# NVIDIA/CUDALibrarySamples

Hardware: NVIDIA H100
Metric: csr_spmv_fp64_effective_hbm_bandwidth (higher is better)
Workload: dtype f64

## Files before the change

### cudalibrarysamples_b200/csrc/spmv_csr_flat.cu

```cuda
#include "spmv_common.cuh"
#include "config.h"
#include "../../include/b200spmv.h"

namespace b200 {

#ifndef B200_FLAT_MIN_CTAS
#define B200_FLAT_MIN_CTAS 10
#endif
#ifndef B200_FLAT_BATCH
#define B200_FLAT_BATCH 4
#endif
#ifndef B200_FLAT_STEPS
#define B200_FLAT_STEPS 8
#endif
#ifndef B200_FLAT_KBLOOP
#define B200_FLAT_KBLOOP (B200_FLAT_STEPS > 8)
#endif
#ifndef B200_FLAT_NZPRE
#define B200_FLAT_NZPRE 0
#endif
constexpr int PLAN_STEPS = 8;
constexpr int PLAN_CHUNK = 32 * PLAN_STEPS;
constexpr int FLAT_STEPS = B200_FLAT_STEPS;
constexpr int FLAT_CHUNK = 32 * FLAT_STEPS;
static_assert(FLAT_STEPS % PLAN_STEPS == 0 && FLAT_STEPS <= 32, "a warp chunk is 1, 2 or 4 plan chunks");
#ifndef B200_FLAT_WARPS
#define B200_FLAT_WARPS 4
#endif
constexpr int FLAT_WARPS = B200_FLAT_WARPS;
constexpr int FLAT_BLOCK = 32 * FLAT_WARPS;
constexpr int FLAT_CTA_NNZ = FLAT_CHUNK * FLAT_WARPS;
constexpr int FLAT_CTA_WORDS = FLAT_CTA_NNZ / 32;
constexpr int FLAT_PAD_NNZ = 2048;
static_assert(FLAT_PAD_NNZ % FLAT_CTA_NNZ == 0, "FLAT_WARPS x FLAT_STEPS must divide 64");
constexpr int FLAT_BATCH64 = B200_FLAT_BATCH;
#ifdef B200_FLAT_BATCH32
constexpr int FLAT_BATCH32 = B200_FLAT_BATCH32;
#else
constexpr int FLAT_BATCH32 = (2 * B200_FLAT_BATCH <= B200_FLAT_STEPS) ? 2 * B200_FLAT_BATCH : B200_FLAT_BATCH;
#endif
constexpr int SCAN_ITEMS = 2048;
static_assert(FLAT_STEPS % FLAT_BATCH64 == 0 && FLAT_STEPS % FLAT_BATCH32 == 0, "steps per chunk must be a multiple of the batch");

struct FlatPlan {
    unsigned* endmask;
    int*      chunk_run;
    int*      nzrow;
    double*   cta_first;
    double*   cta_last;
    int*      cta_flags;
    int*      ctl;
    int*      scratch;
};

static inline size_t flat_align(size_t v) { return (v + 255) / 256 * 256; }
static inline int64_t flat_num_ctas(int64_t nnz) { return (nnz + FLAT_CTA_NNZ - 1) / FLAT_CTA_NNZ; }
static inline int64_t flat_num_chunks_padded(int64_t nnz) { return (nnz + FLAT_PAD_NNZ - 1) / FLAT_PAD_NNZ * (FLAT_PAD_NNZ / PLAN_CHUNK); }

static size_t flat_layout(int64_t rows, int64_t nnz, void* ws, FlatPlan* p) {
    const size_t nchunks = (size_t)flat_num_chunks_padded(nnz);
    const size_t nctas = nchunks;
    const size_t nscan = (size_t)((rows > (int64_t)nchunks ? rows : (int64_t)nchunks) / SCAN_ITEMS + 2);
    size_t o = 0;
    const size_t o_mask = o;  o = flat_align(o + nchunks * PLAN_STEPS * sizeof(unsigned));
    const size_t o_crun = o;  o = flat_align(o + (nchunks + 1) * sizeof(int));
    const size_t o_nzr  = o;  o = flat_align(o + ((size_t)rows + 2 + 32) * sizeof(int));
    const size_t o_cf   = o;  o = flat_align(o + nctas * sizeof(double));
    const size_t o_cl   = o;  o = flat_align(o + nctas * sizeof(double));
    const size_t o_fl   = o;  o = flat_align(o + nctas * sizeof(int));
    const size_t o_ctl  = o;  o = flat_align(o + 64);
    const size_t o_scr  = o;  o = flat_align(o + nscan * sizeof(int));
    if (p) {
        char* b = (char*)ws;
        p->endmask = (unsigned*)(b + o_mask); p->chunk_run = (int*)(b + o_crun); p->nzrow = (int*)(b + o_nzr);
        p->cta_first = (double*)(b + o_cf); p->cta_last = (double*)(b + o_cl); p->cta_flags = (int*)(b + o_fl);
        p->ctl = (int*)(b + o_ctl); p->scratch = (int*)(b + o_scr);
    }
    return o;
}

__global__ void flat_mark_ends_kernel(const int* __restrict__ off, int base, int64_t rows, unsigned* __restrict__ endmask) {
    for (int64_t r = (int64_t)blockIdx.x * blockDim.x + threadIdx.x; r < rows; r += (int64_t)gridDim.x * blockDim.x) {
        const int b = off[r] - base, e = off[r + 1] - base;
        if (e > b) atomicOr(endmask + ((e - 1) >> 5), 1u << ((e - 1) & 31));
    }
}

struct RowNonEmpty {
    const int* off;
    __device__ __forceinline__ int operator()(int64_t r) const { return off[r + 1] > off[r] ? 1 : 0; }
};
struct ChunkEnds {
    const unsigned* endmask;
    __device__ __forceinline__ int operator()(int64_t c) const {
        int n = 0;
#pragma unroll
        for (int k = 0; k < PLAN_STEPS; k++) n += __popc(endmask[c * PLAN_STEPS + k]);
        return n;
    }
};

template <typename V>
__global__ void __launch_bounds__(256) scan_block_sums_kernel(V value, int64_t n, int* __restrict__ block_sums) {
    __shared__ int sw[8];
    const int64_t i0 = (int64_t)blockIdx.x * SCAN_ITEMS;
    int s = 0;
    for (int k = threadIdx.x; k < SCAN_ITEMS; k += 256) {
        const int64_t i = i0 + k;
        s += i < n ? value(i) : 0;
    }
#pragma unroll
    for (int o = 16; o > 0; o >>= 1) s += __shfl_xor_sync(0xffffffffu, s, o);
    if ((threadIdx.x & 31) == 0) sw[threadIdx.x >> 5] = s;
    __syncthreads();
    if (threadIdx.x == 0) {
        int t = 0;
#pragma unroll
        for (int w = 0; w < 8; w++) t += sw[w];
        block_sums[blockIdx.x] = t;
    }
}

__global__ void __launch_bounds__(1024) scan_of_block_sums_kernel(int* __restrict__ block_sums, int64_t nb, int* __restrict__ total) {
    __shared__ int sw[32];
    __shared__ int carry;
    if (threadIdx.x == 0) carry = 0;
    __syncthreads();
    for (int64_t i0 = 0; i0 < nb; i0 += 1024) {
        const int64_t i = i0 + threadIdx.x;
        const int v = i < nb ? block_sums[i] : 0;
        int incl = v;
#pragma unroll
        for (int o = 1; o < 32; o <<= 1) { const int t = __shfl_up_sync(0xffffffffu, incl, o); if ((threadIdx.x & 31) >= o) incl += t; }
        if ((threadIdx.x & 31) == 31) sw[threadIdx.x >> 5] = incl;
        __syncthreads();
        if (threadIdx.x < 32) {
            const int w = sw[threadIdx.x];
            int wi = w;
#pragma unroll
            for (int o = 1; o < 32; o <<= 1) { const int t = __shfl_up_sync(0xffffffffu, wi, o); if (threadIdx.x >= o) wi += t; }
            sw[threadIdx.x] = wi - w;
        }
        __syncthreads();
        const int excl = carry + sw[threadIdx.x >> 5] + incl - v;
        if (i < nb) block_sums[i] = excl;
        __syncthreads();
        if (threadIdx.x == 1023) carry = excl + v;
        __syncthreads();
    }
    if (threadIdx.x == 0) *total = carry;
}

template <typename V, typename E>
__global__ void __launch_bounds__(256) scan_emit_kernel(V value, E emit, int64_t n, const int* __restrict__ block_sums) {
    __shared__ int sw[8];
    __shared__ int carry;
    if (threadIdx.x == 0) carry = block_sums[blockIdx.x];
    __syncthreads();
    const int64_t i0 = (int64_t)blockIdx.x * SCAN_ITEMS;
    for (int k0 = 0; k0 < SCAN_ITEMS; k0 += 256) {
        const int64_t i = i0 + k0 + threadIdx.x;
        const int v = i < n ? value(i) : 0;
        int incl = v;
#pragma unroll
        for (int o = 1; o < 32; o <<= 1) { const int t = __shfl_up_sync(0xffffffffu, incl, o); if ((threadIdx.x & 31) >= o) incl += t; }
        if ((threadIdx.x & 31) == 31) sw[threadIdx.x >> 5] = incl;
        __syncthreads();
        int woff = 0;
#pragma unroll
        for (int w = 0; w < 8; w++) woff += w < (int)(threadIdx.x >> 5) ? sw[w] : 0;
        const int excl = carry + woff + incl - v;
        if (i < n) emit(i, excl, v);
        __syncthreads();
        if (threadIdx.x == 255) carry = excl + v;
        __syncthreads();
    }
}

struct EmitNzRow {
    int* nzrow;
    __device__ __forceinline__ void operator()(int64_t r, int rank, int v) const { if (v) nzrow[rank + 1] = (int)r; }
};
struct EmitChunkRun {
    int* chunk_run;
    __device__ __forceinline__ void operator()(int64_t c, int before, int) const { chunk_run[c] = before; }
};

__global__ void flat_finish_kernel(FlatPlan p, int64_t rows, int64_t nchunks, int64_t nwords) {
    const int nruns = p.ctl[0];
    if (blockIdx.x == 0 && threadIdx.x == 0) {
        p.nzrow[0] = -1;
        p.nzrow[nruns + 1] = (int)rows;
        p.chunk_run[nchunks] = nruns;
        p.ctl[2] = (int)nwords;
    }
    int quiet = 0;
    for (int64_t w = (int64_t)blockIdx.x * blockDim.x + threadIdx.x; w < nwords; w += (int64_t)gridDim.x * blockDim.x)
        quiet += p.endmask[w] == 0u;
#pragma unroll
    for (int o = 16; o > 0; o >>= 1) quiet += __shfl_xor_sync(0xffffffffu, quiet, o);
    if ((threadIdx.x & 31) == 0 && quiet) atomicAdd(p.ctl + 1, quiet);
}

template <typename T>
struct FlatArgs {
    const int* off;
    const int* col;
    const T*   val;
    const T*   x;
    T*         y;
    int        base;
    int        rows;
    int        nnz;
    Scalars<T> s;
    FlatPlan   plan;
};

template <typename T>
__device__ __forceinline__ T flat_allsum(T v) {
#pragma unroll
    for (int o = 16; o > 0; o >>= 1) v += __shfl_xor_sync(0xffffffffu, v, o);
    return v;
}

template <typename T>
__device__ __forceinline__ void flat_store_y(T* yp, T alpha, T v, T beta) {
    T old = T(0);
    if (beta != T(0)) old = *yp;
    *yp = alpha * v + beta * old;
}

template <typename T>
__global__ void __launch_bounds__(FLAT_BLOCK, B200_FLAT_MIN_CTAS) csr_flat_kernel(const FlatArgs<T> a) {
    __shared__ T   sFirst[FLAT_WARPS], sLast[FLAT_WARPS];
    __shared__ int sFrow[FLAT_WARPS];
    __shared__ int sArrived;
    if (threadIdx.x == 0) sArrived = 0;
    __syncthreads();

    const int lane = (int)threadIdx.x & 31, warp = (int)threadIdx.x >> 5;
    const long long c = (long long)blockIdx.x * FLAT_WARPS + warp;
    const long long c0 = c * FLAT_CHUNK;
    const bool active = c0 < a.nnz;
    const T alpha = a.s.a(), beta = a.s.b();
    T   acc = T(0), first = T(0), last = T(0);
    int frow = -1;

    if (active) {
        const int n0 = (int)c0, n1 = min(n0 + FLAT_CHUNK, a.nnz);
        const unsigned mreg = lane < FLAT_STEPS ? __ldg(a.plan.endmask + c * FLAT_STEPS + lane) : 0u;
        int run = __ldg(a.plan.chunk_run + c * (FLAT_STEPS / PLAN_STEPS));
#if B200_FLAT_NZPRE
        const int run0 = run;
        const int nzw = __ldg(a.plan.nzrow + run0 + 1 + lane);
#endif
        const int* colp = a.col + n0;
        const T*   valp = a.val + n0;
        const T*   xp = a.x - a.base;
        constexpr int FLAT_BATCH = sizeof(T) == 8 ? FLAT_BATCH64 : FLAT_BATCH32;
        int cc[FLAT_BATCH];
        T   vv[FLAT_BATCH];
        auto issue = [&](int kb) {
#pragma unroll
            for (int k = 0; k < FLAT_BATCH; k++) {
                const int e = (kb + k) * 32 + lane;
                const bool live = n0 + e < n1;
                cc[k] = live ? ldg_stream(colp + e) : a.base;
                vv[k] = live ? ldg_stream(valp + e) : T(0);
            }
        };
        issue(0);
#if B200_FLAT_KBLOOP
#pragma unroll 1
#else
#pragma unroll
#endif
        for (int kb = 0; kb < FLAT_STEPS; kb += FLAT_BATCH) {
            if (n0 + kb * 32 >= n1) break;
            T p[FLAT_BATCH];
#pragma unroll
            for (int k = 0; k < FLAT_BATCH; k++) p[k] = (n0 + (kb + k) * 32 + lane < n1) ? vv[k] * __ldg(xp + cc[k]) : T(0);
            if (kb + FLAT_BATCH < FLAT_STEPS && n0 + (kb + FLAT_BATCH) * 32 < n1) issue(kb + FLAT_BATCH);
#pragma unroll
            for (int k = 0; k < FLAT_BATCH; k++) {
                const unsigned m = __shfl_sync(0xffffffffu, mreg, kb + k);
                const T pk = p[k];
                if (m == 0u) { acc += pk; continue; }
                const int e1 = __ffs(m) - 1, ek = 31 - __clz(m);
                const bool is_end = (m >> lane) & 1u;
                int row = 0;
#if B200_FLAT_NZPRE
                {
                    const int j = run - run0 + __popc(m & ((1u << lane) - 1u));
                    row = __shfl_sync(0xffffffffu, nzw, j & 31);
                    if (is_end && j >= 32) row = __ldg(a.plan.nzrow + run0 + j + 1);
                }
#else
                if (is_end) row = __ldg(a.plan.nzrow + run + __popc(m & ((1u << lane) - 1u)) + 1);
#endif
                const T t1 = flat_allsum(acc + (lane <= e1 ? pk : T(0)));
                T q = (lane > e1 && lane <= ek) ? pk : T(0);
                if (m & (m - 1u)) {
                    const unsigned below = m & ((1u << lane) - 1u);
                    const int dist = (lane > e1 && lane <= ek) ? lane - (32 - __clz(below)) : 0;
#pragma unroll 1
                    for (int d = 1; d < 32; d <<= 1) {
                        if (__ballot_sync(0xffffffffu, dist >= d) == 0u) break;
                        const T t = __shfl_up_sync(0xffffffffu, q, d);
                        if (dist >= d) q += t;
                    }
                }
                const T res = lane == e1 ? t1 : q;
                bool mine = is_end;
                if (frow < 0) {
                    first = __shfl_sync(0xffffffffu, res, e1);
                    frow = __shfl_sync(0xffffffffu, row, e1);
                    mine = is_end && lane != e1;
                }
                if (mine) flat_store_y(a.y + row, alpha, res, beta);
                run += __popc(m);
                acc = lane > ek ? pk : T(0);
            }
        }
        const int  el = n1 - 1 - n0;
        const unsigned ml = __shfl_sync(0xffffffffu, mreg, el >> 5);
        if (!((ml >> (el & 31)) & 1u)) last = flat_allsum(acc);
    }
    int arrived = 0;
    if (lane == 0) {
        if (frow >= 0) { sFirst[warp] = first; sLast[warp] = last; }
        else           { sFirst[warp] = last;  sLast[warp] = T(0); }
        sFrow[warp] = frow;
        __threadfence_block();
        arrived = atomicAdd(&sArrived, 1);
    }
    if (lane == 0 && arrived == FLAT_WARPS - 1) {
        __threadfence_block();
        const long long cta = blockIdx.x;
        const bool starts_row = cta == 0 || (__ldg(a.plan.endmask + cta * FLAT_CTA_WORDS - 1) >> 31);
        T    running = T(0);
        bool has = false;
#pragma unroll
        for (int w = 0; w < FLAT_WARPS; w++) {
            const int fr = sFrow[w];
            if (fr >= 0) {
                const T tot = running + sFirst[w];
                if (!has && !starts_row) a.plan.cta_first[cta] = (double)tot;
                else flat_store_y(a.y + fr, alpha, tot, beta);
                running = sLast[w];
                has = true;
            } else {
                running += sFirst[w];
            }
        }
        if (!has) { a.plan.cta_first[cta] = (double)running; a.plan.cta_last[cta] = 0.0; }
        else      a.plan.cta_last[cta] = (double)running;
        a.plan.cta_flags[cta] = has ? 1 : 0;
    }
}

template <typename T>
__global__ void __launch_bounds__(256) csr_flat_fixup_kernel(const FlatArgs<T> a, long long nctas) {
    const long long t = (long long)blockIdx.x * blockDim.x + threadIdx.x;
    const T alpha = a.s.a(), beta = a.s.b();
    if (t < a.rows && beta != T(1)) {
        if (__ldg(a.off + t) == __ldg(a.off + t + 1)) flat_store_y(a.y + t, alpha, T(0), beta);
    }
    if (t >= nctas - 1) return;
    const bool tail_open = !(__ldg(a.plan.endmask + (t + 1) * FLAT_CTA_WORDS - 1) >> 31);
    if (!tail_open) return;
    const bool has = __ldcg(a.plan.cta_flags + t) != 0;
    const bool starts_row = t == 0 || (__ldg(a.plan.endmask + t * FLAT_CTA_WORDS - 1) >> 31);
    if (!has && !starts_row) return;
    double sum = has ? __ldcg(a.plan.cta_last + t) : __ldcg(a.plan.cta_first + t);
    long long u = t + 1;
    while (__ldcg(a.plan.cta_flags + u) == 0) { sum += __ldcg(a.plan.cta_first + u); u++; }
    sum += __ldcg(a.plan.cta_first + u);
    const int row = __ldg(a.plan.nzrow + __ldg(a.plan.chunk_run + u * (FLAT_CTA_NNZ / PLAN_CHUNK)) + 1);
    flat_store_y(a.y + row, alpha, (T)sum, beta);
}

template <typename T>
__global__ void flat_scale_y_kernel(T* __restrict__ y, int64_t rows, Scalars<T> s) {
    const T beta = s.b();
    for (int64_t i = (int64_t)blockIdx.x * blockDim.x + threadIdx.x; i < rows; i += (int64_t)gridDim.x * blockDim.x)
        y[i] = beta == T(0) ? T(0) : beta * y[i];
}

template <typename T>
static int launch_flat(cudaStream_t stream, int64_t rows, int64_t nnz, const void* off, const void* col, const void* val, int base,
                       const void* alpha, const void* beta, int on_device, const void* x, void* y, void* ws) {
    FlatArgs<T> a;
    a.off = (const int*)off; a.col = (const int*)col; a.val = (const T*)val; a.x = (const T*)x; a.y = (T*)y;
    a.base = base; a.rows = (int)rows; a.nnz = (int)nnz;
    if (on_device) { a.s.alpha = T(0); a.s.beta = T(0); a.s.alpha_dev = (const T*)alpha; a.s.beta_dev = (const T*)beta; }
    else { a.s.alpha = *(const T*)alpha; a.s.beta = *(const T*)beta; a.s.alpha_dev = nullptr; a.s.beta_dev = nullptr; }
    flat_layout(rows, nnz, ws, &a.plan);
    stats().last_csr_kernel = sizeof(T) == 8 ? "b200::csr_flat_kernel<double>" : "b200::csr_flat_kernel<float>";
    if (nnz == 0) {
        int64_t blocks = (rows + 255) / 256;
        if (blocks > 132 * 16) blocks = 132 * 16;
        flat_scale_y_kernel<T><<<(unsigned)blocks, 256, 0, stream>>>((T*)y, rows, a.s);
        return (int)cudaGetLastError();
    }
    const int64_t nctas = flat_num_ctas(nnz);
    csr_flat_kernel<T><<<(unsigned)nctas, FLAT_BLOCK, 0, stream>>>(a);
    cudaError_t e = cudaGetLastError();
    if (e != cudaSuccess) return (int)e;
    const bool skip_rows = !on_device && *(const T*)beta == T(1);
    const int64_t work = (!skip_rows && rows > nctas - 1) ? rows : (nctas - 1 > 0 ? nctas - 1 : 1);
    csr_flat_fixup_kernel<T><<<(unsigned)((work + 255) / 256), 256, 0, stream>>>(a, (long long)nctas);
    return (int)cudaGetLastError();
}

}

using namespace b200;

extern "C" {

size_t b200spmv_csr_flat_workspace_bytes(int64_t rows, int64_t nnz) {
    if (rows < 0 || nnz < 0) return 0;
    return flat_layout(rows, nnz, nullptr, nullptr);
}

int b200spmv_csr_flat_analyze(void* stream_, int64_t rows, int64_t nnz, const void* row_offsets, int32_t base, void* workspace) {
    if (rows < 0 || nnz < 0 || rows > INT32_MAX - 2 || nnz > INT32_MAX - 65536 || !workspace || (rows > 0 && !row_offsets)) return -1;
    cudaStream_t stream = (cudaStream_t)stream_;
    FlatPlan p;
    const size_t total = flat_layout(rows, nnz, workspace, &p);
    (void)total;
    const int64_t nchunks = flat_num_chunks_padded(nnz), nwords = (nnz + 31) / 32;
    cudaError_t e = cudaMemsetAsync(p.endmask, 0, (size_t)nchunks * PLAN_STEPS * sizeof(unsigned), stream);
    if (e != cudaSuccess) return (int)e;
    e = cudaMemsetAsync(p.ctl, 0, 64, stream);
    if (e != cudaSuccess) return (int)e;
    const int* off = (const int*)row_offsets;
    if (rows > 0) {
        int64_t blocks = (rows + 255) / 256;
        if (blocks > 132 * 32) blocks = 132 * 32;
        flat_mark_ends_kernel<<<(unsigned)blocks, 256, 0, stream>>>(off, base, rows, p.endmask);
        const int64_t nb = (rows + SCAN_ITEMS - 1) / SCAN_ITEMS;
        RowNonEmpty v{off};
        scan_block_sums_kernel<<<(unsigned)nb, 256, 0, stream>>>(v, rows, p.scratch);
        scan_of_block_sums_kernel<<<1, 1024, 0, stream>>>(p.scratch, nb, p.ctl);
        scan_emit_kernel<<<(unsigned)nb, 256, 0, stream>>>(v, EmitNzRow{p.nzrow}, rows, p.scratch);
    }
    if (nchunks > 0) {
        const int64_t nb = (nchunks + SCAN_ITEMS - 1) / SCAN_ITEMS;
        ChunkEnds v{p.endmask};
        scan_block_sums_kernel<<<(unsigned)nb, 256, 0, stream>>>(v, nchunks, p.scratch);
        scan_of_block_sums_kernel<<<1, 1024, 0, stream>>>(p.scratch, nb, p.ctl + 3);
        scan_emit_kernel<<<(unsigned)nb, 256, 0, stream>>>(v, EmitChunkRun{p.chunk_run}, nchunks, p.scratch);
    }
    int64_t fb = (nwords + 255) / 256;
    if (fb > 132 * 8) fb = 132 * 8;
    if (fb < 1) fb = 1;
    flat_finish_kernel<<<(unsigned)fb, 256, 0, stream>>>(p, rows, nchunks, nwords);
    return (int)cudaGetLastError();
}

void b200spmv_csr_flat_plan_offsets(int64_t rows, int64_t nnz, size_t* endmask, size_t* chunk_run, size_t* nzrow, size_t* ctl) {
    FlatPlan p;
    flat_layout(rows, nnz, nullptr, &p);
    if (endmask) *endmask = (size_t)((char*)p.endmask - (char*)nullptr);
    if (chunk_run) *chunk_run = (size_t)((char*)p.chunk_run - (char*)nullptr);
    if (nzrow) *nzrow = (size_t)((char*)p.nzrow - (char*)nullptr);
    if (ctl) *ctl = (size_t)((char*)p.ctl - (char*)nullptr);
}

void b200spmv_csr_flat_params(int32_t* warp_chunk, int32_t* cta_nnz, int32_t* plan_chunk) {
    if (warp_chunk) *warp_chunk = FLAT_CHUNK;
    if (cta_nnz) *cta_nnz = FLAT_CTA_NNZ;
    if (plan_chunk) *plan_chunk = PLAN_CHUNK;
}

int b200spmv_csr_flat_mv(void* stream, int dtype, int64_t rows, int64_t cols, int64_t nnz, const void* row_offsets,
                         const void* col_ind, const void* values, int32_t base, const void* alpha, const void* beta,
                         int scalars_on_device, const void* x, void* y, void* workspace) {
    if (rows < 0 || cols < 0 || nnz < 0 || !alpha || !beta) return -1;
    if (rows == 0) return 0;
    if (!y || !workspace || !row_offsets || (nnz > 0 && (!col_ind || !values || !x))) return -1;
    if (dtype == 0)
        return launch_flat<float>((cudaStream_t)stream, rows, nnz, row_offsets, col_ind, values, base, alpha, beta, scalars_on_device, x, y, workspace);
    if (dtype == 1)
        return launch_flat<double>((cudaStream_t)stream, rows, nnz, row_offsets, col_ind, values, base, alpha, beta, scalars_on_device, x, y, workspace);
    return -1;
}

}
```

Before: 1578.

## Add ring-buffered gather prefetch and PDL launch of the fixup kernel

Replaces the single prefetch batch of col/val loads with a ring of register batches, so loads for later steps are in flight while the current batch gathers x and reduces. The default batch size drops from 4 to 2 with a ring of 2. It also removes the unused NZPRE path. The fixup kernel is now launched with programmatic dependent launch: the empty-row beta scaling overlaps the tail of the main kernel, and griddepcontrol.wait is placed before the cross-CTA carry reads. Risks are higher register pressure from the ring, and a PDL ordering hazard if the empty-row stores race with the main kernel's y writes.

```diff
diff --git a/cudalibrarysamples_b200/csrc/spmv_csr_flat.cu b/cudalibrarysamples_b200/csrc/spmv_csr_flat.cu
--- a/cudalibrarysamples_b200/csrc/spmv_csr_flat.cu
+++ b/cudalibrarysamples_b200/csrc/spmv_csr_flat.cu
@@ -8,16 +8,16 @@
 #define B200_FLAT_MIN_CTAS 10
 #endif
 #ifndef B200_FLAT_BATCH
-#define B200_FLAT_BATCH 4
+#define B200_FLAT_BATCH 2
+#endif
+#ifndef B200_FLAT_RING
+#define B200_FLAT_RING 2
 #endif
 #ifndef B200_FLAT_STEPS
 #define B200_FLAT_STEPS 8
 #endif
 #ifndef B200_FLAT_KBLOOP
 #define B200_FLAT_KBLOOP (B200_FLAT_STEPS > 8)
-#endif
-#ifndef B200_FLAT_NZPRE
-#define B200_FLAT_NZPRE 0
 #endif
 constexpr int PLAN_STEPS = 8;
 constexpr int PLAN_CHUNK = 32 * PLAN_STEPS;
@@ -37,10 +37,13 @@
 #ifdef B200_FLAT_BATCH32
 constexpr int FLAT_BATCH32 = B200_FLAT_BATCH32;
 #else
-constexpr int FLAT_BATCH32 = (2 * B200_FLAT_BATCH <= B200_FLAT_STEPS) ? 2 * B200_FLAT_BATCH : B200_FLAT_BATCH;
-#endif
+constexpr int FLAT_BATCH32 = (2 * B200_FLAT_BATCH * B200_FLAT_RING <= B200_FLAT_STEPS) ? 2 * B200_FLAT_BATCH : B200_FLAT_BATCH;
+#endif
+constexpr int FLAT_RING = B200_FLAT_RING;
 constexpr int SCAN_ITEMS = 2048;
-static_assert(FLAT_STEPS % FLAT_BATCH64 == 0 && FLAT_STEPS % FLAT_BATCH32 == 0, "steps per chunk must be a multiple of the batch");
+static_assert(FLAT_RING >= 2, "a ring of one batch would overwrite the batch whose gathers are in flight");
+static_assert(FLAT_STEPS % (FLAT_RING * FLAT_BATCH64) == 0 && FLAT_STEPS % (FLAT_RING * FLAT_BATCH32) == 0,
+              "steps per chunk must be a multiple of one turn of the ring");
 
 struct FlatPlan {
     unsigned* endmask;
@@ -235,6 +238,7 @@
     __shared__ T   sFirst[FLAT_WARPS], sLast[FLAT_WARPS];
     __shared__ int sFrow[FLAT_WARPS];
     __shared__ int sArrived;
+    asm volatile("griddepcontrol.launch_dependents;" ::: "memory");
     if (threadIdx.x == 0) sArrived = 0;
     __syncthreads();
 
@@ -250,37 +254,38 @@
         const int n0 = (int)c0, n1 = min(n0 + FLAT_CHUNK, a.nnz);
         const unsigned mreg = lane < FLAT_STEPS ? __ldg(a.plan.endmask + c * FLAT_STEPS + lane) : 0u;
         int run = __ldg(a.plan.chunk_run + c * (FLAT_STEPS / PLAN_STEPS));
-#if B200_FLAT_NZPRE
-        const int run0 = run;
-        const int nzw = __ldg(a.plan.nzrow + run0 + 1 + lane);
-#endif
         const int* colp = a.col + n0;
         const T*   valp = a.val + n0;
         const T*   xp = a.x - a.base;
         constexpr int FLAT_BATCH = sizeof(T) == 8 ? FLAT_BATCH64 : FLAT_BATCH32;
-        int cc[FLAT_BATCH];
-        T   vv[FLAT_BATCH];
-        auto issue = [&](int kb) {
+        int cc[FLAT_RING][FLAT_BATCH];
+        T   vv[FLAT_RING][FLAT_BATCH];
+        auto issue = [&](int s, int kb) {
 #pragma unroll
             for (int k = 0; k < FLAT_BATCH; k++) {
                 const int e = (kb + k) * 32 + lane;
                 const bool live = n0 + e < n1;
-                cc[k] = live ? ldg_stream(colp + e) : a.base;
-                vv[k] = live ? ldg_stream(valp + e) : T(0);
+                cc[s][k] = live ? ldg_stream(colp + e) : a.base;
+                vv[s][k] = live ? ldg_stream(valp + e) : T(0);
             }
         };
-        issue(0);
+#pragma unroll
+        for (int s = 0; s + 1 < FLAT_RING; s++) issue(s, s * FLAT_BATCH);
 #if B200_FLAT_KBLOOP
 #pragma unroll 1
 #else
 #pragma unroll
 #endif
-        for (int kb = 0; kb < FLAT_STEPS; kb += FLAT_BATCH) {
+        for (int kr = 0; kr < FLAT_STEPS; kr += FLAT_RING * FLAT_BATCH) {
+#pragma unroll
+        for (int s = 0; s < FLAT_RING; s++) {
+            const int kb = kr + s * FLAT_BATCH;
             if (n0 + kb * 32 >= n1) break;
+            const int kn = kb + (FLAT_RING - 1) * FLAT_BATCH;
+            if (B200_FLAT_KBLOOP || kn < FLAT_STEPS) issue((s + FLAT_RING - 1) % FLAT_RING, kn);
             T p[FLAT_BATCH];
 #pragma unroll
-            for (int k = 0; k < FLAT_BATCH; k++) p[k] = (n0 + (kb + k) * 32 + lane < n1) ? vv[k] * __ldg(xp + cc[k]) : T(0);
-            if (kb + FLAT_BATCH < FLAT_STEPS && n0 + (kb + FLAT_BATCH) * 32 < n1) issue(kb + FLAT_BATCH);
+            for (int k = 0; k < FLAT_BATCH; k++) p[k] = (n0 + (kb + k) * 32 + lane < n1) ? vv[s][k] * __ldg(xp + cc[s][k]) : T(0);
 #pragma unroll
             for (int k = 0; k < FLAT_BATCH; k++) {
                 const unsigned m = __shfl_sync(0xffffffffu, mreg, kb + k);
@@ -289,15 +294,7 @@
                 const int e1 = __ffs(m) - 1, ek = 31 - __clz(m);
                 const bool is_end = (m >> lane) & 1u;
                 int row = 0;
-#if B200_FLAT_NZPRE
-                {
-                    const int j = run - run0 + __popc(m & ((1u << lane) - 1u));
-                    row = __shfl_sync(0xffffffffu, nzw, j & 31);
-                    if (is_end && j >= 32) row = __ldg(a.plan.nzrow + run0 + j + 1);
-                }
-#else
                 if (is_end) row = __ldg(a.plan.nzrow + run + __popc(m & ((1u << lane) - 1u)) + 1);
-#endif
                 const T t1 = flat_allsum(acc + (lane <= e1 ? pk : T(0)));
                 T q = (lane > e1 && lane <= ek) ? pk : T(0);
                 if (m & (m - 1u)) {
@@ -322,6 +319,7 @@
                 acc = lane > ek ? pk : T(0);
             }
         }
+        }
         const int  el = n1 - 1 - n0;
         const unsigned ml = __shfl_sync(0xffffffffu, mreg, el >> 5);
         if (!((ml >> (el & 31)) & 1u)) last = flat_allsum(acc);
@@ -366,6 +364,8 @@
     if (t < a.rows && beta != T(1)) {
         if (__ldg(a.off + t) == __ldg(a.off + t + 1)) flat_store_y(a.y + t, alpha, T(0), beta);
     }
+    if (t >= nctas - 1 && t > 0) return;
+    asm volatile("griddepcontrol.wait;" ::: "memory");
     if (t >= nctas - 1) return;
     const bool tail_open = !(__ldg(a.plan.endmask + (t + 1) * FLAT_CTA_WORDS - 1) >> 31);
     if (!tail_open) return;
@@ -409,8 +409,16 @@
     if (e != cudaSuccess) return (int)e;
     const bool skip_rows = !on_device && *(const T*)beta == T(1);
     const int64_t work = (!skip_rows && rows > nctas - 1) ? rows : (nctas - 1 > 0 ? nctas - 1 : 1);
-    csr_flat_fixup_kernel<T><<<(unsigned)((work + 255) / 256), 256, 0, stream>>>(a, (long long)nctas);
-    return (int)cudaGetLastError();
+    cudaLaunchAttribute pdl;
+    pdl.id = cudaLaunchAttributeProgrammaticStreamSerialization;
+    pdl.val.programmaticStreamSerializationAllowed = 1;
+    cudaLaunchConfig_t cfg = {};
+    cfg.gridDim = dim3((unsigned)((work + 255) / 256));
+    cfg.blockDim = dim3(256);
+    cfg.stream = stream;
+    cfg.attrs = &pdl;
+    cfg.numAttrs = 1;
+    return (int)cudaLaunchKernelEx(&cfg, csr_flat_fixup_kernel<T>, a, (long long)nctas);
 }
 
 }
```

Result: faster. 1624, median of 6 (+2.9%).
